# MechaCritter/Python-Visual-Similarity

Hardware: AMD Instinct MI355X
Metric: images/sec encoded + top-k retrieved, VLAD K256 RootSIFT (higher is better)
Workload: dtype f32

## Files before the change

### include/pvsim.h

```cpp
#ifndef PVSIM_H
#define PVSIM_H

#include <stddef.h>
#include <stdint.h>

#ifdef __cplusplus
extern "C" {
#endif

#define PVS_VERSION 103

typedef enum {
  PVS_OK = 0,
  PVS_ERR_INVALID = 1,
  PVS_ERR_NO_DEVICE = 2,
  PVS_ERR_OOM = 3,
  PVS_ERR_UNSUPPORTED = 4,
  PVS_ERR_DIM = 5,
  PVS_ERR_CAPACITY = 6
} pvs_status;

typedef enum {
  PVS_DESC_F32 = 0,
  PVS_DESC_F32_ROOTSIFT = 1,
  PVS_DESC_U8_ROOTSIFT = 2
} pvs_desc_kind;

typedef enum {
  PVS_OPT_ASSIGN_PREFILTER = 0,
  PVS_OPT_VLAD_PATH = 1,
  PVS_OPT_TOPK_SELECT_ONLY = 2,
  PVS_OPT_AGG_VARIANT = 3,
  PVS_OPT_FISHER_SCALE = 4,
  PVS_OPT_TRAIN_BATCH_CHUNKS = 5,
  PVS_OPT_UPDATE_WINDOW_ROWS = 6,
  PVS_OPT_SQ8_PATH = 7,
  PVS_OPT_GEMM_SLOTS = 8,
  PVS_OPT_COUNT_ = 9
} pvs_option;

typedef struct pvs_ctx pvs_ctx;
typedef struct pvs_codebook pvs_codebook;
typedef struct pvs_gmm pvs_gmm;
typedef struct pvs_pca pvs_pca;
typedef struct pvs_comm pvs_comm;

typedef struct {
  double power_norm_weight;
  double norm_order;
  double epsilon;
} pvs_norm_params;

int pvs_version(void);
const char* pvs_last_error(void);
int pvs_device_count(int* count);
int pvs_init(int device_id, void* stream, pvs_ctx** out);
int pvs_destroy(pvs_ctx* ctx);
int pvs_sync(pvs_ctx* ctx);
void* pvs_stream(pvs_ctx* ctx);
int pvs_device_name(pvs_ctx* ctx, char* buf, size_t buflen);
int pvs_set_option(pvs_ctx* ctx, int option, int value);
int pvs_get_option(pvs_ctx* ctx, int option, int* value);

int pvs_malloc(pvs_ctx* ctx, size_t bytes, void** dptr);
int pvs_free(pvs_ctx* ctx, void* dptr);
int pvs_memcpy_h2d(pvs_ctx* ctx, void* dst_dev, const void* src_host, size_t bytes);
int pvs_memcpy_d2h(pvs_ctx* ctx, void* dst_host, const void* src_dev, size_t bytes);
int pvs_memset(pvs_ctx* ctx, void* dst_dev, int value, size_t bytes);

int pvs_fill_dev(pvs_ctx* ctx, void* dst_dev, int64_t n_elems, int elem_bytes, uint64_t pattern);
int pvs_stream_wait(pvs_ctx* waiter, pvs_ctx* signal);
// ... 287 lines not shown
```

### include/pvsim_diag.h

```cpp
#ifndef PVSIM_DIAG_H
#define PVSIM_DIAG_H

#include "pvsim.h"

#ifdef __cplusplus
extern "C" {
#endif

int pvs_fused_profile(pvs_ctx* ctx, int enable, int64_t* out16);

typedef enum {
  PVS_GEMM_MODEL_EXACT_F32 = 0,
  PVS_GEMM_MODEL_F16_256 = 1,
  PVS_GEMM_MODEL_F16_BOUNDED = 2,
  PVS_GEMM_MODEL_F64 = 3,
  PVS_GEMM_MODEL_F16_2LVL = 4,
  PVS_GEMM_MODEL_GENERIC = 5
} pvs_gemm_model;
typedef enum {
  PVS_GEMM_TAIL_UNSPLIT_BYTES = 1,
  PVS_GEMM_TAIL_UNSPLIT_ONE_SLICE = 2
} pvs_gemm_tail_unsplit;
int pvs_gemm_last_plan(pvs_ctx* ctx, int32_t out12[12]);

#ifdef __cplusplus
}
#endif
#endif
```

### python-visual-similarity_amd/csrc/api.hip

```cpp
#include <algorithm>
#include <cmath>
#include <limits>
#include <memory>

#include "panel_plan.hpp"

namespace pvs {

static thread_local char g_err[512] = "";

void set_error(const char* fmt, ...) {
  va_list ap;
  va_start(ap, fmt);
  vsnprintf(g_err, sizeof(g_err), fmt, ap);
  va_end(ap);
}

static_assert(WS_UPDATE + 1 == pvs_ctx::NWS, "one block per WsSlot");

int ws_reserve(pvs_ctx* ctx, WsSlot which, size_t bytes, void** out) {
  if (bytes == 0) bytes = 16;
  if (ctx->ws_bytes[which] < bytes) {
    if (ctx->ws[which]) {
      PVS_HIP(hipStreamSynchronize(ctx->stream));
// ... 132 lines not shown
  std::unique_ptr<pvs_ctx> c(new pvs_ctx());
  c->device = device_id;
  c->num_cu = prop.multiProcessorCount > 0 ? prop.multiProcessorCount : 256;
  if (stream) {
    c->stream = static_cast<hipStream_t>(stream);
  } else {
    PVS_HIP(hipStreamCreateWithFlags(&c->stream, hipStreamNonBlocking));
    c->owns_stream = true;
  }
  *out = c.release();
  return PVS_OK;
}

PVS_EXPORT int pvs_destroy(pvs_ctx* ctx) {
  if (!ctx) return PVS_OK;
  hipSetDevice(ctx->device);
  hipStreamSynchronize(ctx->stream);
  drain_timers(ctx);
  for (hipEvent_t e : ctx->event_pool) (void)hipEventDestroy(e);
  ctx->event_pool.clear();
  for (auto& kv : ctx->block_cache) (void)hipFree(kv.second);
  ctx->block_cache.clear();
  if (ctx->h_stage) (void)hipHostFree(ctx->h_stage);
  for (int i = 0; i < pvs_ctx::DSIFT_RING; ++i) {
    if (ctx->dsift_h[i]) (void)hipHostFree(ctx->dsift_h[i]);
    if (ctx->dsift_ev[i]) (void)hipEventDestroy(ctx->dsift_ev[i]);
  }
  for (int i = 0; i < pvs_ctx::NWS; ++i)
    if (ctx->ws[i]) hipFree(ctx->ws[i]);
  for (auto& p : ctx->gemm_plan)
    if (p.d_tiles) hipFree(p.d_tiles);
  if (ctx->d_queue) hipFree(ctx->d_queue);
  if (ctx->d_fused_stamps) hipFree(ctx->d_fused_stamps);
  if (ctx->owns_stream) hipStreamDestroy(ctx->stream);
  delete ctx;
  return PVS_OK;
}

PVS_EXPORT int pvs_sync(pvs_ctx* ctx) {
  PVS_NEED(ctx, "ctx");
  PVS_HIP(hipStreamSynchronize(ctx->stream));
  return PVS_OK;
}

PVS_EXPORT void* pvs_stream(pvs_ctx* ctx) { return ctx ? static_cast<void*>(ctx->stream) : nullptr; }

PVS_EXPORT int pvs_device_name(pvs_ctx* ctx, char* buf, size_t buflen) {
  PVS_NEED(ctx, "ctx");
  PVS_NEED(buf, "buf");
  hipDeviceProp_t prop;
  PVS_HIP(hipGetDeviceProperties(&prop, ctx->device));
  snprintf(buf, buflen, "%s (%s, %d CUs)", prop.name, prop.gcnArchName, prop.multiProcessorCount);
  return PVS_OK;
}

PVS_EXPORT int pvs_set_option(pvs_ctx* ctx, int option, int value) {
  PVS_NEED(ctx, "ctx");
  if (option < 0 || option >= PVS_OPT_COUNT_) PVS_FAIL(PVS_ERR_INVALID, "unknown option %d", option);
  const int hi = option == PVS_OPT_GEMM_SLOTS ? 4096 : option == PVS_OPT_UPDATE_WINDOW_ROWS ? (1 << 20) : option == PVS_OPT_TRAIN_BATCH_CHUNKS ? 1024 : option == PVS_OPT_ASSIGN_PREFILTER ? 4 : (option == PVS_OPT_VLAD_PATH || option == PVS_OPT_TOPK_SELECT_ONLY) ? 3 : ((option == PVS_OPT_AGG_VARIANT || option == PVS_OPT_FISHER_SCALE || option == PVS_OPT_SQ8_PATH) ? 2 : 1);
  if (value < 0 || value > hi) PVS_FAIL(PVS_ERR_INVALID, "option %d: value %d out of range 0..%d", option, value, hi);
  ctx->opt[option] = value;
  return PVS_OK;
}
PVS_EXPORT int pvs_get_option(pvs_ctx* ctx, int option, int* value) {
  PVS_NEED(ctx, "ctx");
  PVS_NEED(value, "value");
// ... 965 lines not shown
  PVS_HIP(hipMemcpyAsync(d_indices, h_indices, 8, hipMemcpyHostToDevice, ctx->stream));
  PVS_TRY(launch_kmeanspp_run(ctx, d_x, total_desc, D, n_clusters, trials, d_uni, d_mind, lay.dist(ws), lay.cand(ws), lay.block_sums(ws), lay.small(ws),
                              d_indices));
  PVS_HIP(hipMemcpyAsync(h_indices, d_indices, (size_t)n_clusters * 8, hipMemcpyDeviceToHost, ctx->stream));
  PVS_HIP(hipStreamSynchronize(ctx->stream));
  return PVS_OK;
}

PVS_EXPORT int pvs_fused_profile(pvs_ctx* ctx, int enable, int64_t* out16) {
  PVS_NEED(ctx, "ctx");
  PVS_HIP(hipSetDevice(ctx->device));
  PVS_HIP(hipStreamSynchronize(ctx->stream));
  if (out16) {
    for (int i = 0; i < 16; ++i) out16[i] = 0;
    if (ctx->d_fused_stamps) PVS_HIP(hipMemcpy(out16, ctx->d_fused_stamps, 16 * 8, hipMemcpyDeviceToHost));
  }
  if (enable) {
    if (!ctx->d_fused_stamps) PVS_HIP(hipMalloc(reinterpret_cast<void**>(&ctx->d_fused_stamps), 16 * 8));
    PVS_HIP(hipMemset(ctx->d_fused_stamps, 0, 16 * 8));
  } else if (ctx->d_fused_stamps) {
    PVS_HIP(hipFree(ctx->d_fused_stamps));
    ctx->d_fused_stamps = nullptr;
  }
  return PVS_OK;
}

PVS_EXPORT int pvs_gemm_last_plan(pvs_ctx* ctx, int32_t out12[12]) {
  PVS_NEED(ctx, "ctx");
  PVS_NEED(out12, "out12");
  for (int i = 0; i < 12; ++i) out12[i] = ctx->gemm_last[i];
  return PVS_OK;
}

PVS_EXPORT int pvs_timers_enable(pvs_ctx* ctx, int on) {
  PVS_NEED(ctx, "ctx");
  PVS_TRY(drain_timers(ctx));
  ctx->timers_on = on != 0;
  return PVS_OK;
}
PVS_EXPORT int pvs_timers_reset(pvs_ctx* ctx) {
  PVS_NEED(ctx, "ctx");
  PVS_TRY(drain_timers(ctx));
  for (int i = 0; i < PVS_TIMER_SLOTS; ++i) {
    ctx->t_total[i] = 0;
    ctx->t_count[i] = 0;
  }
  return PVS_OK;
}
PVS_EXPORT int pvs_timers_read(pvs_ctx* ctx, int which, double* total_ms, int64_t* launches) {
  PVS_NEED(ctx, "ctx");
  if (which < 0 || which >= PVS_TIMER_SLOTS) PVS_FAIL(PVS_ERR_INVALID, "timer slot %d out of range", which);
  PVS_TRY(drain_timers(ctx));
  if (total_ms) *total_ms = ctx->t_total[which];
  if (launches) *launches = ctx->t_count[which];
  return PVS_OK;
}
```

### python-visual-similarity_amd/csrc/assign_prefilter.hpp

```cpp
#pragma once

#include "common.hpp"
#include "desc_load.hpp"

namespace pvs {

typedef _Float16 f16x8_t __attribute__((ext_vector_type(8)));
typedef _Float16 f16x4_t __attribute__((ext_vector_type(4)));

constexpr int ASSIGN_THREADS = 512;
constexpr int ASSIGN_ROWS = (ASSIGN_THREADS / 64) * 32;

struct Assign16Args {
  const void* X;
  int64_t total;
  int D, ld;
  const _Float16* C16;
  const float* cnorm;
  int K_pad, D_pad16;
  int c_shift;
  float cmax;
  const _Float16* cnk;
  int cn_e1, K;
  int32_t* labels;
  int64_t* amb_rows;
  unsigned long long* amb_count;
  int64_t cap;
  float2* rowstat;
  unsigned long long* stamps;
  int nprod;
  int shape16;
};

int launch_assign16x(pvs_ctx* ctx, const Assign16Args& p, int kind, size_t lds, int grid);

__device__ __forceinline__ void pf_fill_sqrt_table(uint32_t* lds_t) {
  if (threadIdx.x < 256) {
    const float sv = sqrtf((float)threadIdx.x);
    const _Float16 hi = (_Float16)sv, lo = (_Float16)(sv - (float)hi);
    lds_t[threadIdx.x] = (uint32_t)__builtin_bit_cast(unsigned short, hi) | ((uint32_t)__builtin_bit_cast(unsigned short, lo) << 16);
  }
}
__device__ __forceinline__ void pf_u8_fragment(const uint32_t* lds_t, const uint32_t* xw, f16x8_t* xh, f16x8_t* xl) {
  uint32_t hw[4], lw[4];
#pragma unroll
  for (int i = 0; i < 2; ++i)
#pragma unroll
    for (int pq = 0; pq < 2; ++pq) {
      const uint32_t w = xw[i];
      const uint32_t e0 = lds_t[(w >> (16 * pq)) & 0xffu], e1 = lds_t[(w >> (16 * pq + 8)) & 0xffu];
      hw[2 * i + pq] = __builtin_amdgcn_perm(e1, e0, 0x05040100u);
      lw[2 * i + pq] = __builtin_amdgcn_perm(e1, e0, 0x07060302u);
    }
  *xh = __builtin_bit_cast(f16x8_t, make_uint4(hw[0], hw[1], hw[2], hw[3]));
  *xl = __builtin_bit_cast(f16x8_t, make_uint4(lw[0], lw[1], lw[2], lw[3]));
}

template <int KIND, int NP, bool LUT>
__device__ __forceinline__ float prefilter_eps(float nx, float cmax, float lut_sd, float sqrt_d) {
  const float xc = nx * cmax;
  constexpr float conv_err = DescTraits<KIND>::rootsift ? 4.8e-7f : 0.f;
  const float cc = LUT ? cmax * cmax * lut_sd : cmax * cmax;
  constexpr float drop_err = (3 - NP) * 4.9e-4f;
  return 2.f * (4.8e-7f + 2.4e-7f + 4.8e-5f + 7.7e-6f + 1e-9f + conv_err + drop_err) * xc * (1.f + sqrt_d * 1e-9f) + (LUT ? 6.0e-7f : 2.4e-7f) * (cc + 2.f * xc);
}

__device__ __forceinline__ void pf_label_or_list(const Assign16Args& a, bool settled, bool leader, int64_t row, int bidx, int lane,
// ... 16 lines not shown
```

### python-visual-similarity_amd/csrc/common.hpp

```cpp
#pragma once
#include <hip/hip_runtime.h>

#include <cmath>
#include <cstdarg>
#include <cstdint>
#include <cstdio>
#include <cstring>
#include <map>
#include <type_traits>
#include <vector>

#include "../../include/pvsim.h"
#include "../../include/pvsim_diag.h"
#include "workspace.hpp"

#define PVS_EXPORT extern "C" __attribute__((visibility("default")))

namespace pvs {

void set_error(const char* fmt, ...);

#define PVS_FAIL(code, ...)        \
  do {                             \
    ::pvs::set_error(__VA_ARGS__); \
// ... 17 lines not shown
  } while (0)

#define PVS_NEED(p, what) \
  if (!(p)) PVS_FAIL(PVS_ERR_INVALID, "%s: null %s", __func__, what)
#define PVS_ALIGNED(p, a, what) \
  if (reinterpret_cast<uintptr_t>(p) % (a)) PVS_FAIL(PVS_ERR_INVALID, "%s: %s must be %d-byte aligned", __func__, what, (int)(a))

constexpr int WAVE = 64;

enum TimerSlot { T_ASSIGN = 0, T_AGGREGATE = 1, T_GEMM = 2, T_TOPK = 3, T_FPOST = 4, T_FMOM = 5, T_MISC = 6, T_RESCORE = 7 };

struct TimerRec {
  hipEvent_t a, b;
  int slot;
};

}

struct pvs_ctx {
  int device = 0;
  hipStream_t stream = nullptr;
  bool owns_stream = false;
  int num_cu = 256;
  static constexpr int NWS = 18;
  void* ws[NWS] = {};
  size_t ws_bytes[NWS] = {};
  struct GemmPlanSlot {
    int key[4] = {-1, -1, -1, -1};
    int n_main = 0, n_tail = 0, splitk = 1;
    void* d_tiles = nullptr;
    size_t cap = 0;
  } gemm_plan[5];
  std::map<const void*, int> lds_attr;
  int opt[PVS_OPT_COUNT_] = {1, 0, 0, 0, 0, 0, 0, 0, 0};
  int32_t gemm_last[12] = {-1, -1, -1, -1, -1, -1, -1, -1, -1, -1, -1, -1};
  unsigned int* d_queue = nullptr;
  unsigned long long* d_fused_stamps = nullptr;
  bool timers_on = false;
  std::vector<pvs::TimerRec> pending;
  std::vector<hipEvent_t> event_pool;
  std::multimap<size_t, void*> block_cache;
  std::map<void*, size_t> block_size;
  size_t block_cache_bytes = 0;
  void* h_stage = nullptr;
  size_t h_stage_bytes = 0;
  static constexpr int DSIFT_RING = 4;
  void* dsift_h[DSIFT_RING] = {};
  size_t dsift_h_bytes[DSIFT_RING] = {};
  hipEvent_t dsift_ev[DSIFT_RING] = {};
  int dsift_next = 0;
  double t_total[PVS_TIMER_SLOTS] = {0};
  int64_t t_count[PVS_TIMER_SLOTS] = {0};
};

struct pvs_codebook {
  int K = 0, D = 0;
  int K_pad = 0, D_pad = 0;
  float* d_cent = nullptr;
  float* d_cpad = nullptr;
  float* d_cnorm = nullptr;
  void* d_c16 = nullptr;
  int D_pad16 = 0;
  int c16_shift = 0;
  float cmax = 0.f;
  void* d_cnk = nullptr;
  void* d_c16n = nullptr;
  int cn_e1 = 0;
};
// ... 161 lines not shown
```

### python-visual-similarity_amd/csrc/vlad.hip

```cpp
#include "assign_prefilter.hpp"

namespace pvs {

typedef float f32x16 __attribute__((ext_vector_type(16)));

struct AssignArgs {
  const void* X;
  int64_t total;
  int D, ld;
  const float* Cpad;
  const float* cnorm;
  int K_pad, D_pad;
  int32_t* labels;
  const int64_t* rows;
  const unsigned long long* nrows;
  int64_t rows_cap;
};

constexpr int ASSIGN_DCHUNK = 128;

template <int NT, int KIND, bool VEC>
__global__ __launch_bounds__(ASSIGN_THREADS, 2) void assign_kernel(AssignArgs a) {
  extern __shared__ __attribute__((aligned(16))) char smem[];
  constexpr int CB = 32 * NT;
  const int cw_max = a.D_pad < ASSIGN_DCHUNK ? a.D_pad : ASSIGN_DCHUNK;
  const int stride = cw_max + 4;
  float* lds_c = reinterpret_cast<float*>(smem);
  float* lds_n = lds_c + CB * stride;

  const int lane = threadIdx.x & 63, wave = threadIdx.x >> 6;
  const int j = lane & 31, h = lane >> 5;
  const int ncb = a.K_pad / CB;
  const int nsc = (a.D_pad + ASSIGN_DCHUNK - 1) / ASSIGN_DCHUNK;
  const bool restage = (ncb * nsc) > 1;
  const int64_t n_items = a.rows ? (int64_t)a.nrows[blockIdx.x] : a.total;
  const int64_t nblocks = (n_items + ASSIGN_ROWS - 1) / ASSIGN_ROWS;
  const int64_t* const my_rows = a.rows ? a.rows + (int64_t)blockIdx.x * a.rows_cap : nullptr;

  auto stage = [&](int cb, int sc) {
    const int cw = min(ASSIGN_DCHUNK, a.D_pad - sc * ASSIGN_DCHUNK);
    const int c4n = cw >> 2;
    for (int idx = threadIdx.x; idx < CB * c4n; idx += ASSIGN_THREADS) {
      const int r = idx / c4n, c4 = idx - r * c4n;
      const float4 v = *reinterpret_cast<const float4*>(a.Cpad + (int64_t)(cb * CB + r) * a.D_pad +
                                                        sc * ASSIGN_DCHUNK + 4 * c4);
      *reinterpret_cast<float4*>(lds_c + r * stride + 4 * c4) = v;
    }
    for (int idx = threadIdx.x; idx < CB; idx += ASSIGN_THREADS) lds_n[idx] = a.cnorm[cb * CB + idx];
  };

  if (!restage) {
    stage(0, 0);
    __syncthreads();
  }

  for (int64_t blk = my_rows ? 0 : blockIdx.x; blk < nblocks; blk += my_rows ? 1 : gridDim.x) {
    const int64_t item = blk * ASSIGN_ROWS + wave * 32 + j;
    const bool rvalid = item < n_items;
    const int64_t row = (my_rows && rvalid) ? my_rows[item] : item;
    float best = INFINITY;
    int bidx = 0;

// ... 485 lines not shown
}

int assign_tiles_for(int K) {
  const int k32 = (K + 31) / 32 * 32;
  return k32 > 128 ? 8 : (k32 > 64 ? 4 : (k32 > 32 ? 2 : 1));
}

int launch_assign(pvs_ctx* ctx, const pvs_codebook* cb, const void* d_desc, int kind, int64_t total, int ld,
                  int32_t* d_labels, const float2** rowstat_out) {
  if (rowstat_out) *rowstat_out = nullptr;
  if (total <= 0) return PVS_OK;
  const bool rs = kind != PVS_DESC_F32;
  if (rs && cb->D > ASSIGN_DCHUNK)
    PVS_FAIL(PVS_ERR_UNSUPPORTED, "fused RootSIFT needs D <= %d (got %d)", ASSIGN_DCHUNK, cb->D);
  const int nt = assign_tiles_for(cb->K);
  if (cb->K_pad % (32 * nt) != 0) PVS_FAIL(PVS_ERR_INVALID, "codebook padding does not match the tile count");
  AssignArgs a{d_desc, total, cb->D, ld, cb->d_cpad, cb->d_cnorm, cb->K_pad, cb->D_pad, d_labels, nullptr, nullptr, 0};
  const int esz = kind == PVS_DESC_U8_ROOTSIFT ? 1 : 4;
  const bool vec = (cb->D % 4 == 0) && (ld % 4 == 0) && ((reinterpret_cast<uintptr_t>(d_desc) % (4 * esz)) == 0);
  const int cw = cb->D_pad < ASSIGN_DCHUNK ? cb->D_pad : ASSIGN_DCHUNK;
  const size_t lds = (size_t)(32 * nt) * (cw + 4) * 4 + (size_t)(32 * nt) * 4;
  const int64_t nblocks = (total + ASSIGN_ROWS - 1) / ASSIGN_ROWS;
  const int grid = (int)(nblocks < ctx->num_cu ? nblocks : ctx->num_cu);
  ScopedTimer tm(ctx, T_ASSIGN);
  const bool pre = cb->d_c16 != nullptr && total >= 4096 && ctx->opt[PVS_OPT_ASSIGN_PREFILTER] != 0;
  if (pre) {
    const int64_t cap = (nblocks + grid - 1) / grid * ASSIGN_ROWS;
    char* ws = nullptr;
    const bool stat = rowstat_out != nullptr && kind == PVS_DESC_U8_ROOTSIFT;
    WsLayout<> lay;
    const auto cnt_p = lay.add<unsigned long long>((size_t)grid);
    const auto rows_p = lay.add<int64_t>((size_t)grid * cap);
    const auto stat_p = lay.add<float2>(stat ? (size_t)total : 0);
    PVS_TRY(ws_reserve(ctx, WS_LISTS, lay.bytes(), &ws));
    unsigned long long* cnt = cnt_p(ws);
    int64_t* rows = rows_p(ws);
    float2* rowstat = stat ? stat_p(ws) : nullptr;
    if (stat) *rowstat_out = rowstat;
    Assign16Args p{d_desc, total, cb->D, ld, static_cast<const _Float16*>(cb->d_c16), cb->d_cnorm, cb->K_pad, cb->D_pad16,
                   cb->c16_shift, cb->cmax, static_cast<const _Float16*>(cb->d_cnk), cb->cn_e1, cb->K, d_labels, rows, cnt, cap, rowstat,
                   ctx->d_fused_stamps, ctx->opt[PVS_OPT_ASSIGN_PREFILTER] == 2 ? 2 : (ctx->opt[PVS_OPT_ASSIGN_PREFILTER] == 3 ? 1 : 3),
                   ctx->opt[PVS_OPT_ASSIGN_PREFILTER] == 4 ? 1 : 0};
    const size_t lds16 = (size_t)2 * cb->K_pad * (128 + 8) * 2 + (size_t)cb->K_pad * 4 + (size_t)cb->K_pad * 8 + 1024;
    PVS_TRY(launch_assign16(ctx, p, kind, cb->K_pad / 32, vec, lds16, grid));
    a.rows = rows;
    a.nrows = cnt;
    a.rows_cap = cap;
  }
  return dispatch_desc_kind(kind, [&](auto k) { return launch_assign_kind<decltype(k)::value>(ctx, a, nt, vec, lds, grid); });
}

struct AggArgs {
  const void* X;
  int D, ld;
  const int64_t* offsets;
  const int32_t* labels;
  const float* cent;
  int K;
  float power, eps;
  int norm_mode;
  float norm_p;
  float* out;
  float* inv_norm;
  const float2* rowstat;
};

constexpr int AGG_THREADS = 256;
constexpr int AGG_WAVES = AGG_THREADS / 64;
constexpr int AGG_CHUNK = 4096;

template <int KIND, int GROUP, int VW, int NREG, bool HIOCC = false>
__global__ __launch_bounds__(AGG_THREADS, (HIOCC ? 8 : 1)) void vlad_aggregate_kernel(AggArgs a) {
  extern __shared__ __attribute__((aligned(16))) char smem[];
  const int K = a.K, D = a.D;
  int* hist = reinterpret_cast<int*>(smem);
  int* start = hist + AGG_WAVES * K;
  float* rowsq = reinterpret_cast<float*>(start + K + 1);
  int* scan_tmp = reinterpret_cast<int*>(rowsq + K);
  uint16_t* order = reinterpret_cast<uint16_t*>(scan_tmp + AGG_WAVES);

// ... 487 lines not shown
```

### python-visual-similarity_amd/pvsim/_ffi.py

```python
from __future__ import annotations

import ctypes as C
import os
import threading

import numpy as np

from ._errors import CapacityError

_HERE = os.path.dirname(os.path.abspath(__file__))
LIB_PATH = os.environ.get("PVSIM_LIB", os.path.join(_HERE, "libpvsim_hip.so"))

PVS_OK, PVS_ERR_INVALID, PVS_ERR_NO_DEVICE, PVS_ERR_OOM, PVS_ERR_UNSUPPORTED, PVS_ERR_DIM, PVS_ERR_CAPACITY = range(7)
_EXC = {PVS_ERR_INVALID: ValueError, PVS_ERR_NO_DEVICE: RuntimeError, PVS_ERR_OOM: MemoryError,
        PVS_ERR_UNSUPPORTED: NotImplementedError, PVS_ERR_DIM: RuntimeError, PVS_ERR_CAPACITY: CapacityError}

DESC_F32, DESC_F32_ROOTSIFT, DESC_U8_ROOTSIFT = 0, 1, 2
OPT_ASSIGN_PREFILTER, OPT_VLAD_PATH, OPT_TOPK_SELECT_ONLY, OPT_AGG_VARIANT, OPT_FISHER_SCALE = 0, 1, 2, 3, 4
OPT_TRAIN_BATCH_CHUNKS = 5
PIX_U8_RGB, PIX_U8_GRAY, PIX_F32_RGB, PIX_F32_GRAY = 0, 1, 2, 3
DSIFT_U8, DSIFT_F32, DSIFT_F32_RAW, DSIFT_F32_QUANT = 0, 1, 2, 3
OPT_UPDATE_WINDOW_ROWS = 6
OPT_SQ8_PATH = 7
OPT_GEMM_SLOTS = 8
GEMM_EXACT_F32, GEMM_F16_256, GEMM_F16_BOUNDED, GEMM_F64, GEMM_F16_2LVL, GEMM_GENERIC = range(6)
GEMM_TAIL_UNSPLIT_BYTES, GEMM_TAIL_UNSPLIT_ONE_SLICE = 1, 2
GEMM_PLAN_FIELDS = ("model", "tiles_m", "tiles_n", "symm", "dual", "n_main", "n_tail", "split", "nparts", "tail_unsplit",
                    "main_8ph", "accumulate")
SQ8_PATH_AUTO, SQ8_PATH_ROWS, SQ8_PATH_MATRIX = 0, 1, 2
SQ8_MAX_L = 131072
RANGE_UPPER = 1
RANGE_PATH_AUTO, RANGE_PATH_EXACT, RANGE_PATH_FILTERED = 0, 1, 2
RANGE_MAX_CAPACITY = 1 << 40
SUBSET_PATH_AUTO, SUBSET_PATH_MASK, SUBSET_PATH_LISTED = 0, 1, 2
SUBSET_MAX_K = 1024
SCAN_TILE = 2048
COMBINE_CHUNK_BYTES, COMBINE_BATCH = 8192, 8
DIFFUSE_DOT_BLOCK, DIFFUSE_MAX_COLUMNS = 256, 65536
KRR_MAX_K1, KRR_MAX_KQ = 64, 1024
VLAD_PATH_AUTO, VLAD_PATH_GATHER, VLAD_PATH_STREAM, VLAD_PATH_FUSED = 0, 1, 2, 3
TIMER_NAMES = ("assign", "aggregate", "cosine_gemm", "topk", "fisher_posterior", "fisher_moments", "misc", "rescore")


class NormParams(C.Structure):
    _fields_ = [("power_norm_weight", C.c_double), ("norm_order", C.c_double), ("epsilon", C.c_double)]


_vp, _i64, _int, _sz = C.c_void_p, C.c_int64, C.c_int, C.c_size_t
_pp = C.POINTER(C.c_void_p)
_np = C.POINTER(NormParams)

SIGNATURES = {
    "pvs_version": [],
    "pvs_last_error": [],
    "pvs_device_count": [C.POINTER(C.c_int)],
    "pvs_init": [_int, _vp, _pp],
    "pvs_destroy": [_vp],
# ... 98 lines not shown
    "pvs_graph_lists_dev": [_vp, _vp, _vp, _i64, _int, _i64, _vp, _i64, _vp, _vp],
    "pvs_graph_merge_dev": [_vp, _vp, _vp, _vp, _vp, _i64, _int, _int, _i64, _i64, _vp, _vp],
    "pvs_graph_damage_dev": [_vp, _vp, _i64, _int, _vp, _vp],
    "pvs_graph_remap_dev": [_vp, _vp, _i64, _int, _vp, _vp, _vp],
    "pvs_graph_gather_rows_dev": [_vp, _vp, _i64, _i64, _vp, _i64, _vp],
    "pvs_graph_affinity_sim_dev": [_vp, _vp, _i64, _int, _int, _vp],
    "pvs_krr_sets_dev": [_vp, _vp, _i64, _int, _int, _vp, _vp],
    "pvs_krr_members_dev": [_vp, _vp, _vp, _vp, _i64, _int, _vp, _vp],
    "pvs_krr_weights_dev": [_vp, _vp, _vp, _i64, _int, _int, _vp, _vp],
    "pvs_krr_expand_dev": [_vp, _vp, _vp, _vp, _i64, _int, _int, _vp, _vp, _vp],
    "pvs_krr_query_dev": [_vp, _vp, _vp, _vp, _vp, _vp, _i64, _int, _int, _int, _int, _vp, _vp, _i64, _int, _vp, _vp, _vp, _vp],
    "pvs_krr_score_dev": [_vp, _vp, _vp, _vp, _vp, _i64, _int, _vp, _vp, _vp, _vp, _i64, _int, _int, C.c_double, _vp],
    "pvs_asmk_aggregate_dev": [_vp, _vp, _vp, _int, _vp, _vp, _i64, _i64, _vp, _vp, _int, _vp, _vp, _vp],
    "pvs_asmk_aggregate_ma_dev": [_vp, _vp, _vp, _int, _vp, _vp, _i64, _i64, _vp, _int, _vp, _int, _vp, _vp, _vp],
    "pvs_asmk_score_dev": [_vp, _i64, _vp, _vp, _vp, _int, _int, _vp, _vp, _vp, _i64, _vp, _vp, _vp, _vp, _int, _vp, _i64],
    "pvs_asmk_invert_dev": [_vp, _int, _int, _vp, _vp, _i64, _vp, _vp, _vp, _i64, _int, _vp, _vp, _vp],
    "pvs_asmk_weight_sums_dev": [_vp, _int, _vp, _vp, _i64, _vp, _vp, _vp, _vp],
    "pvs_asmk_insert_dev": [_vp, _int, _int, _vp, _vp, _vp, _vp, _vp, _vp, _vp, _vp, _vp, _vp, _vp],
    "pvs_asmk_remove_dev": [_vp, _int, _int, _i64, _vp, _vp, _vp, _vp, _vp, _vp, _vp, _vp, _vp],
    "pvs_asmk_expand_dev": [_vp, _i64, _vp, _vp, _vp, _int, _int, _vp, _vp, _vp, _i64, _int, _vp, _vp, _int, _int, _int, _vp, _int, _int,
                            _vp, _vp, _vp, _vp],
    "pvs_sq8_encode_dev": [_vp, _vp, _i64, _int, _vp, _vp],
    "pvs_sq8_topk_dev": [_vp, _vp, _vp, _i64, _vp, _vp, _i64, _int, _int, _i64, _int, _vp, _vp],
    "pvs_cosine_range_dev": [_vp, _vp, _i64, _vp, _i64, _i64, _vp, _vp, C.c_float, _int, _int, _int, _i64, _vp, _vp, _vp, _vp, _vp],
    "pvs_pair_components_dev": [_vp, _vp, _vp, _i64, _i64, _vp, _vp],
    "pvs_subset_create": [_vp, _vp, _i64, _i64, _pp],
    "pvs_subset_destroy": [_vp, _vp],
    "pvs_cosine_topk_subset_dev": [_vp, _vp, _i64, _vp, _i64, _i64, _vp, _vp, _vp, _int, _int, _int, _vp, _vp, _vp],
    "pvs_sq8_topk_subset_dev": [_vp, _vp, _vp, _i64, _vp, _vp, _i64, _int, _vp, _int, _int, _int, _vp, _vp, _vp],
    "pvs_ivf_sq8_scan_topk_dev": [_vp, _vp, _vp, _i64, _int, _vp, _int, _vp, _vp, _int, _vp, _vp, _vp, _int, _int, _vp, _vp],
    "pvs_ivf_sq8_scan_plan": [_vp, _i64, _int, _vp, _int, _int, _vp],
    "pvs_fused_profile": [_vp, _int, _vp],
    "pvs_gemm_last_plan": [_vp, _vp],
    "pvs_timers_enable": [_vp, _int],
    "pvs_timers_reset": [_vp],
    "pvs_timers_read": [_vp, _int, C.POINTER(C.c_double), C.POINTER(C.c_int64)],
}

_lib = None
_lock = threading.Lock()


def mapped_hip_runtimes() -> list[str]:
    found = []
    try:
        with open("/proc/self/maps") as f:
            for line in f:
                path = line.rsplit(None, 1)[-1] if "/" in line else ""
                if "libamdhip64" in os.path.basename(path) and path not in found:
                    found.append(path)
    except OSError:
        pass
    return found


def _one_hip_runtime() -> None:
    if mapped_hip_runtimes():
        return
    import importlib.util
    try:
        spec = importlib.util.find_spec("torch")
    except (ImportError, ValueError):
        spec = None
    for loc in (spec.submodule_search_locations if spec and spec.submodule_search_locations else []):
        cand = os.path.join(loc, "lib", "libamdhip64.so")
        if os.path.exists(cand):
# ... 46 lines not shown
```

### python-visual-similarity_amd/pvsim/asmk.py

```python
from __future__ import annotations

import math

import numpy as np

from ._ffi import DESC_F32, DESC_F32_ROOTSIFT, DESC_U8_ROOTSIFT

__all__ = ["ASMKIndex", "ASMKExpansion", "selectivity", "word_weights", "gammas", "random_projection"]

SCALE = 1023
IDF_SCALE = 64
MAX_ROWS = 8192
MAX_MA = 8
MAX_KEYS = 16384
PANEL_BYTES = 64 << 20
MAX_MEMBERS = 32
MAX_QUERY_VOTE = 65535
EXPAND_BYTES = 256 << 20
PAD_BYTE = 0x7F
_KIND = "asmk_index"


def selectivity(bits: int, alpha: float = 3.0, tau: float = 0.0) -> np.ndarray:
    if bits not in (32, 64, 96, 128):
# ... 363 lines not shown
                wt = word_weights(np.diff(word_off), N, idf) if weights is None else weights
                dev["wt"] = ctx.buffer(wt.nbytes).upload(wt)
                gamma = _gammas_of_sums(got["sums"](dev["wt"].ptr))
                dev["word_off"], dev["ent_img"], dev["ent_sig"] = tmp.keep(got["d_word_off"]), tmp.keep(got["d_img"]), tmp.keep(got["d_sig"])
            dev["gamma_db"] = ctx.buffer(gamma.nbytes).upload(gamma) if N else ctx.buffer(0)
            dev["sel"] = ctx.buffer(sel.nbytes).upload(sel)
            dev["projection"] = None if projection is None else ctx.buffer(projection.nbytes).upload(projection)
        except Exception:
            for b in dev.values():
                if b is not None:
                    (b.close if b is cb else b.free)()
            raise
        self = cls(local.paths, cent, word_off, None, None, gamma, wt, sel, bits, alpha, tau, idf, projection, desc_kind, ctx, extractor,
                   weights is not None)
        self._dev, self._cap_e, self._cap_n = dev, got["total"], N
        return self

    @classmethod
    def fit(cls, local, n_words: int, train_rows: int | None = None, random_state=0, max_iter: int = 20, **build_kwargs) -> "ASMKIndex":
        from . import learn
        total = local.total_rows
        if isinstance(n_words, bool) or int(n_words) != n_words or not (1 <= n_words <= 65536):
            raise ValueError(f"n_words must be an integer in 1..65536, got {n_words!r}")
        if total < n_words:
            raise ValueError(f"{total} rows cannot train {n_words} words")
        want = min(total, 64 * int(n_words)) if train_rows is None else int(train_rows)
        if not (n_words <= want <= total):
            raise ValueError(f"train_rows must lie in n_words..{total}, got {train_rows!r}")
        kind = build_kwargs.get("desc_kind", DESC_U8_ROOTSIFT)
        ctx = local.ctx
        keep = np.zeros(total, np.uint8)
        keep[np.random.RandomState(random_state).permutation(total)[:want]] = 1
        with ctx.scratch() as tmp:
            stage, out, d_keep, d_pos = tmp(want * 128), tmp(want * 128 * 4), tmp.upload(keep), tmp((total + 1) * 8)
            ctx.keep_positions_dev(d_keep.ptr, total, d_pos.ptr)
            ctx.compact_rows_dev(local.rows.ptr, total, 128, d_keep.ptr, d_pos.ptr, stage.ptr)
            ctx.materialise_dev(stage.ptr, kind, 128, want, out.ptr)
            ctx.sync()
            model = learn.fit_kmeans(learn.DeviceRows(ctx, want, 128, out), int(n_words), max_iter=max_iter, random_state=random_state)
        return cls.build(local, model, random_state=random_state, **build_kwargs)

    def __len__(self) -> int:
        return len(self._paths)

    @property
    def paths(self) -> list:
        return list(self._paths)

    @property
    def n_words(self) -> int:
        return self.centroids.shape[0]

    def list_sizes(self) -> np.ndarray:
        return np.diff(self.word_off)

    @property
    def ctx(self):
        if self._ctx is None:
            from .engine import default_context
            self._ctx = default_context()
        return self._ctx

    @property
    def extractor(self):
        if self._extractor is None:
            from .features import KeypointRootSIFT
            self._extractor = KeypointRootSIFT(nfeatures=2000, ctx=self._ctx)
# ... 397 lines not shown
```

### python-visual-similarity_amd/pvsim/engine.py

```python
from __future__ import annotations

import ctypes as C
import os
import sys
import threading

import numpy as np

from . import _ffi
from ._ffi import DESC_F32, DESC_F32_ROOTSIFT, DESC_U8_ROOTSIFT, check, norm_params, ptr

__all__ = ["Context", "default_context", "pack_descriptors", "dsift_count", "dsift_frames", "sift_workspace", "diffuse_workspace", "DESC_F32", "DESC_F32_ROOTSIFT", "DESC_U8_ROOTSIFT"]


def pack_descriptors(desc_list, dim: int, dtype=np.float32):
    counts = [0 if d is None else int(d.shape[0]) for d in desc_list]
    offsets = np.zeros(len(desc_list) + 1, dtype=np.int64)
    np.cumsum(counts, out=offsets[1:])
    packed = np.empty((int(offsets[-1]), dim), dtype=dtype)
    for d, o in zip(desc_list, offsets[:-1]):
        if d is not None and d.shape[0]:
            if d.shape[1] != dim:
                raise RuntimeError(f"descriptor dimension {d.shape[1]} does not match the model input dimension {dim}")
            packed[o:o + d.shape[0]] = d
# ... 200 lines not shown

    def sync(self):
        check(_ffi.lib().pvs_sync(self.handle))

    @property
    def stream(self) -> int:
        return int(_ffi.lib().pvs_stream(self.handle) or 0)

    def set_option(self, option: int, value: int) -> None:
        check(_ffi.lib().pvs_set_option(self.handle, int(option), int(value)))

    def get_option(self, option: int) -> int:
        v = C.c_int()
        check(_ffi.lib().pvs_get_option(self.handle, int(option), C.byref(v)))
        return int(v.value)

    def option(self, option: int, value: int):
        ctx = self

        class _Scoped:
            def __enter__(self_inner):
                self_inner.old = ctx.get_option(option)
                ctx.set_option(option, value)

            def __exit__(self_inner, *exc):
                ctx.set_option(option, self_inner.old)

        return _Scoped()

    def gemm_last_plan(self) -> dict:
        out = (C.c_int32 * 12)()
        check(_ffi.lib().pvs_gemm_last_plan(self.handle, out))
        return dict(zip(_ffi.GEMM_PLAN_FIELDS, (int(v) for v in out)))

    def fill_dev(self, d_ptr: int, n_elems: int, dtype: str, value) -> None:
        a = np.array([value], dtype=dtype)
        if a.itemsize not in (4, 8):
            raise ValueError("fill_dev: 4- or 8-byte element types only")
        pattern = int(a.view(np.uint32 if a.itemsize == 4 else np.uint64)[0])
        check(_ffi.lib().pvs_fill_dev(self.handle, ptr(d_ptr), int(n_elems), a.itemsize, C.c_uint64(pattern)))

    def wait_for(self, other: "Context") -> None:
        check(_ffi.lib().pvs_stream_wait(self.handle, other.handle))

    def device_name(self) -> str:
        buf = C.create_string_buffer(256)
        check(_ffi.lib().pvs_device_name(self.handle, buf, 256))
        return buf.value.decode()

    def codebook(self, centroids) -> Codebook:
        c = np.ascontiguousarray(centroids, dtype=np.float32)
        if c.ndim != 2:
            raise ValueError("centroids must be (K, D)")
        h = C.c_void_p()
        check(_ffi.lib().pvs_codebook_create(self.handle, ptr(c), c.shape[0], c.shape[1], C.byref(h)))
        cb = Codebook(self, h)
        cb.K, cb.D = c.shape
        return cb

    def gmm(self, weights, means, covariances) -> GMM:
        w = np.ascontiguousarray(weights, dtype=np.float64)
        m = np.ascontiguousarray(means, dtype=np.float64)
        v = np.ascontiguousarray(covariances, dtype=np.float64)
        if m.ndim != 2 or v.shape != m.shape or w.shape != (m.shape[0],):
            raise ValueError("GMM tables must be weights (K,), means (K, D), diagonal covariances (K, D)")
        h = C.c_void_p()
# ... 630 lines not shown
```

Measured before the change: 418,900.

## Add near-candidate assignment pass that resolves most rows before exact fallback

Adds a new kernel, enabled by default for D=128, that scores each listed row against all centroids with fp16 MFMA. It keeps the candidates that fall within an error bound of the best, rescores those candidates exactly in f32, and writes the label directly. Rows with too many candidates or non-finite scaling go to a fallback list, and the existing exact assign kernel then runs only on those rows. The aim is to skip the expensive exact prefilter path for most descriptors, at the cost of an extra pass and more workspace. The change also adds a stats query, and a Python scratch-size edit grows the compaction stage buffer to the total row count.

```diff
diff --git a/include/pvsim.h b/include/pvsim.h
--- a/include/pvsim.h
+++ b/include/pvsim.h
@@ -35,8 +35,9 @@
   PVS_OPT_TRAIN_BATCH_CHUNKS = 5,
   PVS_OPT_UPDATE_WINDOW_ROWS = 6,
   PVS_OPT_SQ8_PATH = 7,
-  PVS_OPT_GEMM_SLOTS = 8,
-  PVS_OPT_COUNT_ = 9
+  PVS_OPT_ASSIGN_NEAR = 8,
+  PVS_OPT_GEMM_SLOTS = 9,
+  PVS_OPT_COUNT_ = 10
 } pvs_option;
 
 typedef struct pvs_ctx pvs_ctx;
diff --git a/include/pvsim_diag.h b/include/pvsim_diag.h
--- a/include/pvsim_diag.h
+++ b/include/pvsim_diag.h
@@ -23,6 +23,8 @@
 } pvs_gemm_tail_unsplit;
 int pvs_gemm_last_plan(pvs_ctx* ctx, int32_t out12[12]);
 
+int pvs_assign_last_stats(pvs_ctx* ctx, int64_t out4[4]);
+
 #ifdef __cplusplus
 }
 #endif
diff --git a/python-visual-similarity_amd/csrc/api.hip b/python-visual-similarity_amd/csrc/api.hip
--- a/python-visual-similarity_amd/csrc/api.hip
+++ b/python-visual-similarity_amd/csrc/api.hip
@@ -188,6 +188,7 @@
     if (p.d_tiles) hipFree(p.d_tiles);
   if (ctx->d_queue) hipFree(ctx->d_queue);
   if (ctx->d_fused_stamps) hipFree(ctx->d_fused_stamps);
+  if (ctx->d_assign_stats) hipFree(ctx->d_assign_stats);
   if (ctx->owns_stream) hipStreamDestroy(ctx->stream);
   delete ctx;
   return PVS_OK;
@@ -1219,6 +1220,20 @@
   return PVS_OK;
 }
 
+PVS_EXPORT int pvs_assign_last_stats(pvs_ctx* ctx, int64_t out4[4]) {
+  PVS_NEED(ctx, "ctx");
+  PVS_NEED(out4, "out4");
+  const int mode = ctx->assign_last_mode;
+  out4[0] = mode == 2 ? -1 : 0; out4[1] = 0; out4[2] = 0; out4[3] = mode == 2 ? -1 : 0;
+  if (mode != 1) return PVS_OK;
+  PVS_HIP(hipSetDevice(ctx->device));
+  PVS_HIP(hipStreamSynchronize(ctx->stream));
+  std::vector<unsigned long long> h((size_t)ctx->assign_last_grid * 4);
+  PVS_HIP(hipMemcpy(h.data(), ctx->d_assign_stats, h.size() * sizeof(unsigned long long), hipMemcpyDeviceToHost));
+  for (size_t i = 0; i < h.size(); ++i) out4[i & 3] += (int64_t)h[i];
+  return PVS_OK;
+}
+
 PVS_EXPORT int pvs_timers_enable(pvs_ctx* ctx, int on) {
   PVS_NEED(ctx, "ctx");
   PVS_TRY(drain_timers(ctx));
diff --git a/python-visual-similarity_amd/csrc/assign_near.hip b/python-visual-similarity_amd/csrc/assign_near.hip
--- /dev/null
+++ b/python-visual-similarity_amd/csrc/assign_near.hip
@@ -0,0 +1,274 @@
+#include "assign_prefilter.hpp"
+
+namespace pvs {
+
+typedef float f32x16 __attribute__((ext_vector_type(16)));
+
+constexpr int NEAR_THREADS = 256;
+constexpr int NEAR_ROWS = (NEAR_THREADS / 64) * 32;
+constexpr int NEAR_ROW_CAP = 16;
+constexpr int NEAR_TSTRIDE = 128 + 8;
+constexpr int NEAR_XSTRIDE = 128 + 4;
+constexpr int NEAR_ENT = 32 * NEAR_ROW_CAP;
+
+size_t assign_near_lds(int K_pad) {
+  return (size_t)K_pad * NEAR_TSTRIDE * 2 + (size_t)K_pad * 8 + (size_t)NEAR_ROWS * NEAR_XSTRIDE * 4 + (size_t)(NEAR_THREADS / 64) * NEAR_ENT * 8;
+}
+
+template <int KIND>
+__global__ __launch_bounds__(NEAR_THREADS) void assign_near_kernel(AssignNearArgs a) {
+  extern __shared__ __attribute__((aligned(16))) char smem[];
+  __shared__ unsigned int s_fb, s_done, s_entries;
+  const int lane = threadIdx.x & 63, wave = threadIdx.x >> 6;
+  const int j = lane & 31, h = lane >> 5;
+  const int64_t n_items = (int64_t)a.nrows[blockIdx.x];
+  if (n_items == 0) {
+    if (threadIdx.x == 0) {
+      a.fb_count[blockIdx.x] = 0ull;
+      unsigned long long* st = a.stats + 4 * (size_t)blockIdx.x;
+      st[0] = 0ull; st[1] = 0ull; st[2] = 0ull; st[3] = 0ull;
+    }
+    return;
+  }
+  _Float16* lds_h = reinterpret_cast<_Float16*>(smem);
+  _Float16* lds_k = lds_h + (size_t)a.K_pad * NEAR_TSTRIDE;
+  float* lds_x = reinterpret_cast<float*>(lds_k + 4 * (size_t)a.K_pad);
+  int* lds_e = reinterpret_cast<int*>(lds_x + NEAR_ROWS * NEAR_XSTRIDE) + wave * NEAR_ENT;
+  float* lds_v = reinterpret_cast<float*>(reinterpret_cast<int*>(lds_x + NEAR_ROWS * NEAR_XSTRIDE) + (NEAR_THREADS / 64) * NEAR_ENT) + wave * NEAR_ENT;
+  float* my_x = lds_x + wave * 32 * NEAR_XSTRIDE;
+
+  for (int idx = threadIdx.x; idx < a.K_pad * 16; idx += NEAR_THREADS) {
+    const int r = idx >> 4, c8 = idx & 15;
+    *reinterpret_cast<uint4*>(lds_h + r * NEAR_TSTRIDE + 8 * c8) = *reinterpret_cast<const uint4*>(a.C16 + (int64_t)r * 128 + 8 * c8);
+  }
+  for (int idx = threadIdx.x; idx < a.K_pad; idx += NEAR_THREADS)
+    *reinterpret_cast<uint2*>(lds_k + 4 * idx) = *reinterpret_cast<const uint2*>(a.cnk + 4 * idx);
+  if (threadIdx.x == 0) { s_fb = 0u; s_done = 0u; s_entries = 0u; }
+  __syncthreads();
+
+  const int64_t* const my_rows = a.rows + (int64_t)blockIdx.x * a.rows_cap;
+  int64_t* const my_fb = a.fb_rows + (int64_t)blockIdx.x * a.rows_cap;
+  const int64_t nblocks = (n_items + NEAR_ROWS - 1) / NEAR_ROWS;
+  const int ntiles = a.K_pad >> 5;
+  const float sqrt_d = sqrtf(128.f);
+  uint32_t valid16 = 0u;
+#pragma unroll
+  for (int r = 0; r < 16; ++r)
+    if (8 * (r >> 2) + 4 * h + (r & 3) < (a.K & 31)) valid16 |= 1u << r;
+
+  auto row_of = [&](int64_t blk_) {
+    const int64_t item = blk_ * NEAR_ROWS + wave * 32 + j;
+    return my_rows[item < n_items ? item : n_items - 1];
+  };
+  float4 xb[16];
+  auto request_rows = [&](int64_t r) {
+#pragma unroll
+    for (int t = 0; t < 16; ++t) xb[t] = load4<KIND>(a.X, r, a.ld, 8 * t + 4 * h);
+  };
+  int64_t row = row_of(0);
+  int64_t row_next = nblocks > 1 ? row_of(1) : row;
+  request_rows(row);
+
+  for (int64_t blk = 0; blk < nblocks; ++blk) {
+    const bool rvalid = blk * NEAR_ROWS + wave * 32 + j < n_items;
+    if constexpr (DescTraits<KIND>::rootsift) {
+      float s = 0.f;
+#pragma unroll
+      for (int t = 0; t < 16; ++t) s += (xb[t].x + xb[t].y) + (xb[t].z + xb[t].w);
+      s += __shfl_xor(s, 32, 64);
+      const RootsiftRow<KIND> rr(s);
+#pragma unroll
+      for (int t = 0; t < 16; ++t) {
+        xb[t].x = rr(xb[t].x);
+        xb[t].y = rr(xb[t].y);
+        xb[t].z = rr(xb[t].z);
+        xb[t].w = rr(xb[t].w);
+      }
+    }
+    float n2 = 0.f, amax = 0.f;
+#pragma unroll
+    for (int t = 0; t < 16; ++t) {
+      *reinterpret_cast<float4*>(my_x + j * NEAR_XSTRIDE + 8 * t + 4 * h) = xb[t];
+      n2 = fmaf(xb[t].x, xb[t].x, n2); n2 = fmaf(xb[t].y, xb[t].y, n2);
+      n2 = fmaf(xb[t].z, xb[t].z, n2); n2 = fmaf(xb[t].w, xb[t].w, n2);
+      amax = fmaxf(amax, fmaxf(fmaxf(fabsf(xb[t].x), fabsf(xb[t].y)), fmaxf(fabsf(xb[t].z), fabsf(xb[t].w))));
+    }
+    n2 += __shfl_xor(n2, 32, 64);
+    amax = fmaxf(amax, __shfl_xor(amax, 32, 64));
+    const float nx = sqrtf(n2) * 1.0001f;
+    int ex = 13;
+    if (amax > 0.f) (void)frexpf(amax, &ex);
+    int x_shift = 13 - ex;
+    bool finite = nx <= 3.0e38f;
+    if (x_shift > 40 || x_shift < -40) { finite = false; x_shift = 0; }
+    if (x_shift + a.cn_e1 < -14 || x_shift + a.cn_e1 > 15) finite = false;
+    const float xs = ldexpf(1.f, x_shift);
+    f16x8_t xh[8];
+#pragma unroll
+    for (int t = 0; t < 8; ++t) {
+      xh[t][0] = (_Float16)(xb[2 * t].x * xs); xh[t][1] = (_Float16)(xb[2 * t].y * xs);
+      xh[t][2] = (_Float16)(xb[2 * t].z * xs); xh[t][3] = (_Float16)(xb[2 * t].w * xs);
+      xh[t][4] = (_Float16)(xb[2 * t + 1].x * xs); xh[t][5] = (_Float16)(xb[2 * t + 1].y * xs);
+      xh[t][6] = (_Float16)(xb[2 * t + 1].z * xs); xh[t][7] = (_Float16)(xb[2 * t + 1].w * xs);
+    }
+    const int64_t row_cur = row;
+    __builtin_amdgcn_sched_barrier(0);
+    if (blk + 1 < nblocks) {
+      request_rows(row_next);
+      row = row_next;
+      if (blk + 2 < nblocks) row_next = row_of(blk + 2);
+    }
+    __builtin_amdgcn_sched_barrier(0);
+
+    f16x8_t cnb;
+    {
+      const _Float16 pw = (h == 0 && finite) ? (_Float16)ldexpf(1.f, x_shift + a.cn_e1) : (_Float16)0.f;
+#pragma unroll
+      for (int q = 0; q < 8; ++q) cnb[q] = (_Float16)0.f;
+      cnb[0] = pw; cnb[1] = pw; cnb[2] = pw;
+    }
+    f32x16 acc[8];
+    f16x8_t fa[2][8];
+    auto fetch = [&](int buf, int tile) {
+#pragma unroll
+      for (int t = 0; t < 8; ++t)
+        fa[buf][t] = *reinterpret_cast<const f16x8_t*>(lds_h + (32 * tile + j) * NEAR_TSTRIDE + 16 * t + 8 * h);
+    };
+    fetch(0, 0);
+#pragma unroll
+    for (int tile = 0; tile < 8; ++tile) {
+#pragma unroll
+      for (int r = 0; r < 16; ++r) acc[tile][r] = 0.f;
+      if (tile < ntiles) {
+        if (tile + 1 < ntiles) fetch((tile + 1) & 1, tile + 1);
+        const f16x4_t pk = *reinterpret_cast<const f16x4_t*>(lds_k + 4 * (32 * tile + j));
+        __builtin_amdgcn_sched_barrier(0);
+#pragma unroll
+        for (int t = 0; t < 8; ++t) acc[tile] = __builtin_amdgcn_mfma_f32_32x32x16_f16(fa[tile & 1][t], xh[t], acc[tile], 0, 0, 0);
+        f16x8_t ca;
+#pragma unroll
+        for (int q = 0; q < 8; ++q) ca[q] = (_Float16)0.f;
+        if (h == 0) { ca[0] = pk[0]; ca[1] = pk[1]; ca[2] = pk[2]; }
+        acc[tile] = __builtin_amdgcn_mfma_f32_32x32x16_f16(ca, cnb, acc[tile], 0, 0, 0);
+        __builtin_amdgcn_sched_barrier(0);
+      }
+    }
+    float smax = -INFINITY;
+#pragma unroll
+    for (int tile = 0; tile < 8; ++tile) {
+      if (32 * tile + 32 <= a.K) {
+#pragma unroll
+        for (int r = 0; r < 16; ++r) smax = fmaxf(smax, acc[tile][r]);
+      } else if (32 * tile < a.K) {
+#pragma unroll
+        for (int r = 0; r < 16; ++r) smax = fmaxf(smax, ((valid16 >> r) & 1u) ? acc[tile][r] : -INFINITY);
+      }
+    }
+    smax = fmaxf(smax, __shfl_xor(smax, 32, 64));
+    const float m2s = -2.f * ldexpf(1.f, -(x_shift + a.c_shift));
+    const float best = smax * m2s;
+    const float eps = prefilter_eps<KIND, 1, false>(nx, a.cmax, 1.f, sqrt_d);
+    const float thr = best + 2.f * eps;
+    const bool usable = finite && fabsf(best) <= 3.0e38f;
+    uint32_t m[4] = {0u, 0u, 0u, 0u};
+#pragma unroll
+    for (int tile = 0; tile < 8; ++tile) {
+      uint32_t mm = 0u;
+      if (32 * tile + 32 <= a.K) {
+#pragma unroll
+        for (int r = 0; r < 16; ++r) mm |= (acc[tile][r] * m2s <= thr) ? (1u << r) : 0u;
+      } else if (32 * tile < a.K) {
+#pragma unroll
+        for (int r = 0; r < 16; ++r) mm |= (acc[tile][r] * m2s <= thr) ? (1u << r) : 0u;
+        mm &= valid16;
+      }
+      m[tile >> 1] |= mm << (16 * (tile & 1));
+      __builtin_amdgcn_sched_barrier(0);
+    }
+    const int n_mine = __popc(m[0]) + __popc(m[1]) + __popc(m[2]) + __popc(m[3]);
+    const int n_other = __shfl_xor(n_mine, 32, 64);
+    const int n_row = n_mine + n_other;
+    const bool take = rvalid && usable && n_row >= 1 && n_row <= NEAR_ROW_CAP;
+    int incl = (take && h == 0) ? n_row : 0;
+#pragma unroll
+    for (int d = 1; d < 32; d <<= 1) {
+      const int o = __shfl_up(incl, d, 64);
+      if (lane >= d) incl += o;
+    }
+    const int E = __shfl(incl, 31, 64);
+    const int rbase = __shfl(incl, j, 64) - (take ? n_row : 0);
+    if (take) {
+      int e = rbase + (h == 0 ? 0 : n_other);
+#pragma unroll
+      for (int w = 0; w < 4; ++w) {
+        uint32_t bits = m[w];
+        while (bits != 0u) {
+          const int b = __builtin_ctz(bits);
+          bits &= bits - 1u;
+          const int tile = 2 * w + (b >> 4), r = b & 15;
+          lds_e[e++] = (j << 16) | (32 * tile + 8 * (r >> 2) + 4 * h + (r & 3));
+        }
+      }
+    }
+    __syncthreads();
+    for (int e0 = 0; e0 < E; e0 += 64) {
+      const int e = e0 + lane;
+      const int ent = e < E ? lds_e[e] : 0;
+      const int k = ent & 0xffff;
+      const float* xr = my_x + (ent >> 16) * NEAR_XSTRIDE;
+      const float* cr = a.Cpad + (size_t)k * a.D_pad;
+      float4 cv[32];
+#pragma unroll
+      for (int q = 0; q < 32; ++q) cv[q] = *reinterpret_cast<const float4*>(cr + 4 * q);
+      const float cnk = a.cnorm[k];
+      __builtin_amdgcn_sched_barrier(0);
+      float dot = 0.f;
+#pragma unroll
+      for (int t = 0; t < 16; ++t) {
+        const float4 xa = *reinterpret_cast<const float4*>(xr + 8 * t), xc = *reinterpret_cast<const float4*>(xr + 8 * t + 4);
+        const float4 ca = cv[2 * t], cc = cv[2 * t + 1];
+        dot = fmaf(ca.x, xa.x, dot); dot = fmaf(cc.x, xc.x, dot);
+        dot = fmaf(ca.y, xa.y, dot); dot = fmaf(cc.y, xc.y, dot);
+        dot = fmaf(ca.z, xa.z, dot); dot = fmaf(cc.z, xc.z, dot);
+        dot = fmaf(ca.w, xa.w, dot); dot = fmaf(cc.w, xc.w, dot);
+      }
+      if (e < E) lds_v[e] = fmaf(-2.f, dot, cnk);
+    }
+    __syncthreads();
+    if (take && h == 0) {
+      float bv = INFINITY;
+      int bk = 0x7fffffff;
+      for (int i = 0; i < n_row; ++i) {
+        const float v = lds_v[rbase + i];
+        const int k = lds_e[rbase + i] & 0xffff;
+        if (v < INFINITY && (v < bv || (v == bv && k < bk))) { bv = v; bk = k; }
+      }
+      a.labels[row_cur] = bv < INFINITY ? bk : 0;
+    }
+    const bool fb = rvalid && !take && h == 0;
+    const unsigned long long fmask = __ballot(fb), tmask = __ballot(take && h == 0);
+    unsigned int base = 0;
+    if (lane == 0) {
+      if (fmask != 0ull) base = atomicAdd(&s_fb, (unsigned int)__popcll(fmask));
+      if (tmask != 0ull) atomicAdd(&s_done, (unsigned int)__popcll(tmask));
+      if (E != 0) atomicAdd(&s_entries, (unsigned int)E);
+    }
+    base = __shfl(base, 0, 64);
+    if (fb) my_fb[base + __popcll(fmask & ((1ull << lane) - 1ull))] = row_cur;
+    __syncthreads();
+  }
+  if (threadIdx.x == 0) {
+    a.fb_count[blockIdx.x] = s_fb;
+    unsigned long long* st = a.stats + 4 * (size_t)blockIdx.x;
+    st[0] = (unsigned long long)n_items; st[1] = s_done; st[2] = s_entries; st[3] = s_fb;
+  }
+}
+
+int launch_assign_near(pvs_ctx* ctx, const AssignNearArgs& p, int kind, int grid) {
+  const size_t lds = assign_near_lds(p.K_pad);
+  return dispatch_desc_kind(kind, [&](auto k) {
+    return launch_lds(ctx, assign_near_kernel<decltype(k)::value>, dim3(grid), dim3(NEAR_THREADS), lds, p);
+  });
+}
+
+}
diff --git a/python-visual-similarity_amd/csrc/assign_prefilter.hpp b/python-visual-similarity_amd/csrc/assign_prefilter.hpp
--- a/python-visual-similarity_amd/csrc/assign_prefilter.hpp
+++ b/python-visual-similarity_amd/csrc/assign_prefilter.hpp
@@ -33,6 +33,26 @@
 };
 
 int launch_assign16x(pvs_ctx* ctx, const Assign16Args& p, int kind, size_t lds, int grid);
+
+struct AssignNearArgs {
+  const void* X;
+  int ld;
+  const _Float16* C16;
+  const _Float16* cnk;
+  const float* Cpad;
+  const float* cnorm;
+  int K, K_pad, D_pad;
+  int c_shift, cn_e1;
+  float cmax;
+  int32_t* labels;
+  const int64_t* rows;
+  const unsigned long long* nrows;
+  int64_t rows_cap;
+  int64_t* fb_rows;
+  unsigned long long* fb_count;
+  unsigned long long* stats;
+};
+int launch_assign_near(pvs_ctx* ctx, const AssignNearArgs& p, int kind, int grid);
 
 __device__ __forceinline__ void pf_fill_sqrt_table(uint32_t* lds_t) {
   if (threadIdx.x < 256) {
diff --git a/python-visual-similarity_amd/csrc/common.hpp b/python-visual-similarity_amd/csrc/common.hpp
--- a/python-visual-similarity_amd/csrc/common.hpp
+++ b/python-visual-similarity_amd/csrc/common.hpp
@@ -73,8 +73,10 @@
     size_t cap = 0;
   } gemm_plan[5];
   std::map<const void*, int> lds_attr;
-  int opt[PVS_OPT_COUNT_] = {1, 0, 0, 0, 0, 0, 0, 0, 0};
+  int opt[PVS_OPT_COUNT_] = {1, 0, 0, 0, 0, 0, 0, 0, 0, 0};
   int32_t gemm_last[12] = {-1, -1, -1, -1, -1, -1, -1, -1, -1, -1, -1, -1};
+  unsigned long long* d_assign_stats = nullptr;
+  int assign_last_mode = 0, assign_last_grid = 0;
   unsigned int* d_queue = nullptr;
   unsigned long long* d_fused_stamps = nullptr;
   bool timers_on = false;
diff --git a/python-visual-similarity_amd/csrc/vlad.hip b/python-visual-similarity_amd/csrc/vlad.hip
--- a/python-visual-similarity_amd/csrc/vlad.hip
+++ b/python-visual-similarity_amd/csrc/vlad.hip
@@ -28,6 +28,7 @@
   float* lds_c = reinterpret_cast<float*>(smem);
   float* lds_n = lds_c + CB * stride;
 
+  if (a.rows != nullptr && a.nrows[blockIdx.x] == 0ull) return;
   const int lane = threadIdx.x & 63, wave = threadIdx.x >> 6;
   const int j = lane & 31, h = lane >> 5;
   const int ncb = a.K_pad / CB;
@@ -579,6 +580,8 @@
     const auto cnt_p = lay.add<unsigned long long>((size_t)grid);
     const auto rows_p = lay.add<int64_t>((size_t)grid * cap);
     const auto stat_p = lay.add<float2>(stat ? (size_t)total : 0);
+    const auto fb_cnt_p = lay.add<unsigned long long>((size_t)grid);
+    const auto fb_rows_p = lay.add<int64_t>((size_t)grid * cap);
     PVS_TRY(ws_reserve(ctx, WS_LISTS, lay.bytes(), &ws));
     unsigned long long* cnt = cnt_p(ws);
     int64_t* rows = rows_p(ws);
@@ -593,6 +596,21 @@
     a.rows = rows;
     a.nrows = cnt;
     a.rows_cap = cap;
+    ctx->assign_last_mode = 2;
+    if (vec && cb->D == 128 && cb->D_pad16 == 128 && cb->D_pad == 128 && ctx->opt[PVS_OPT_ASSIGN_NEAR] == 0) {
+      if (ctx->d_assign_stats == nullptr)
+        PVS_HIP(hipMalloc(reinterpret_cast<void**>(&ctx->d_assign_stats), (size_t)ctx->num_cu * 4 * sizeof(unsigned long long)));
+      AssignNearArgs q{d_desc, ld, static_cast<const _Float16*>(cb->d_c16), static_cast<const _Float16*>(cb->d_cnk), cb->d_cpad, cb->d_cnorm,
+                       cb->K, cb->K_pad, cb->D_pad, cb->c16_shift, cb->cn_e1, cb->cmax, d_labels, rows, cnt, cap, fb_rows_p(ws), fb_cnt_p(ws),
+                       ctx->d_assign_stats};
+      PVS_TRY(launch_assign_near(ctx, q, kind, grid));
+      a.rows = q.fb_rows;
+      a.nrows = q.fb_count;
+      ctx->assign_last_mode = 1;
+      ctx->assign_last_grid = grid;
+    }
+  } else {
+    ctx->assign_last_mode = 0;
   }
   return dispatch_desc_kind(kind, [&](auto k) { return launch_assign_kind<decltype(k)::value>(ctx, a, nt, vec, lds, grid); });
 }
diff --git a/python-visual-similarity_amd/pvsim/_ffi.py b/python-visual-similarity_amd/pvsim/_ffi.py
--- a/python-visual-similarity_amd/pvsim/_ffi.py
+++ b/python-visual-similarity_amd/pvsim/_ffi.py
@@ -22,7 +22,8 @@
 DSIFT_U8, DSIFT_F32, DSIFT_F32_RAW, DSIFT_F32_QUANT = 0, 1, 2, 3
 OPT_UPDATE_WINDOW_ROWS = 6
 OPT_SQ8_PATH = 7
-OPT_GEMM_SLOTS = 8
+OPT_ASSIGN_NEAR = 8
+OPT_GEMM_SLOTS = 9
 GEMM_EXACT_F32, GEMM_F16_256, GEMM_F16_BOUNDED, GEMM_F64, GEMM_F16_2LVL, GEMM_GENERIC = range(6)
 GEMM_TAIL_UNSPLIT_BYTES, GEMM_TAIL_UNSPLIT_ONE_SLICE = 1, 2
 GEMM_PLAN_FIELDS = ("model", "tiles_m", "tiles_n", "symm", "dual", "n_main", "n_tail", "split", "nparts", "tail_unsplit",
@@ -187,6 +188,7 @@
     "pvs_ivf_sq8_scan_plan": [_vp, _i64, _int, _vp, _int, _int, _vp],
     "pvs_fused_profile": [_vp, _int, _vp],
     "pvs_gemm_last_plan": [_vp, _vp],
+    "pvs_assign_last_stats": [_vp, _vp],
     "pvs_timers_enable": [_vp, _int],
     "pvs_timers_reset": [_vp],
     "pvs_timers_read": [_vp, _int, C.POINTER(C.c_double), C.POINTER(C.c_int64)],
diff --git a/python-visual-similarity_amd/pvsim/asmk.py b/python-visual-similarity_amd/pvsim/asmk.py
--- a/python-visual-similarity_amd/pvsim/asmk.py
+++ b/python-visual-similarity_amd/pvsim/asmk.py
@@ -419,7 +419,7 @@
         keep = np.zeros(total, np.uint8)
         keep[np.random.RandomState(random_state).permutation(total)[:want]] = 1
         with ctx.scratch() as tmp:
-            stage, out, d_keep, d_pos = tmp(want * 128), tmp(want * 128 * 4), tmp.upload(keep), tmp((total + 1) * 8)
+            stage, out, d_keep, d_pos = tmp(total * 128), tmp(want * 128 * 4), tmp.upload(keep), tmp((total + 1) * 8)
             ctx.keep_positions_dev(d_keep.ptr, total, d_pos.ptr)
             ctx.compact_rows_dev(local.rows.ptr, total, 128, d_keep.ptr, d_pos.ptr, stage.ptr)
             ctx.materialise_dev(stage.ptr, kind, 128, want, out.ptr)
diff --git a/python-visual-similarity_amd/pvsim/engine.py b/python-visual-similarity_amd/pvsim/engine.py
--- a/python-visual-similarity_amd/pvsim/engine.py
+++ b/python-visual-similarity_amd/pvsim/engine.py
@@ -256,6 +256,11 @@
         out = (C.c_int32 * 12)()
         check(_ffi.lib().pvs_gemm_last_plan(self.handle, out))
         return dict(zip(_ffi.GEMM_PLAN_FIELDS, (int(v) for v in out)))
+
+    def assign_last_stats(self) -> dict:
+        out = (C.c_int64 * 4)()
+        check(_ffi.lib().pvs_assign_last_stats(self.handle, out))
+        return dict(zip(("listed", "labelled", "entries", "fallback"), (int(v) for v in out)))
 
     def fill_dev(self, d_ptr: int, n_elems: int, dtype: str, value) -> None:
         a = np.array([value], dtype=dtype)
```

New measurement: 419,600 (median of 4 runs). No clear change (+0.2%).
